# MCG-NJU/MotionRAG

Hardware: AMD Instinct MI355X
Metric: denoise_step_frames_per_sec (higher is better)
Workload: dtype bf16

## Files before the change

### motionrag_amd/csrc/gemm_w4.hip

```cpp
#include "gemm_common.h"

namespace {

__device__ __forceinline__ int lane_id_here() {
  int l;
  asm volatile("v_mbcnt_lo_u32_b32 %0, -1, 0\n\tv_mbcnt_hi_u32_b32 %0, -1, %0" : "=v"(l));
  return l;
}
__device__ __forceinline__ int opaque_sign(int x) {
  asm volatile("" : "+v"(x));
  return x;
}

template <int EPI>
__device__ __forceinline__ void epilogue_w4(const GemmP& p, char* smem, f32x4 (&acc)[8][8], const long long bm0, const long long bn0, const int wave, const int wrow0,
                                            const int wcol0, const long long Mend) {
  constexpr bool HAS_R = (EPI == MRAG_EPI_GATE_RESID || EPI == MRAG_EPI_RESID), HAS_G = (EPI == MRAG_EPI_GATE_RESID), QK = (EPI == MRAG_EPI_QKNORM_ROPE);
  const int lane = lane_id_here();
  const int frag_row = opaque_sign(lane & 15), frag_q = lane >> 4;
  const long long n0 = bn0 + wcol0 + frag_q * 4;
  const long long m0 = bm0 + wrow0;
  long long g_b = 0, g_pos = 0;
  if constexpr (HAS_G || QK) {
    g_b = m0 / p.rows_per_batch;
    g_pos = m0 - g_b * p.rows_per_batch;
  }
  if (m0 >= Mend || bn0 + wcol0 >= p.N) return;
  const int mrows = (int)(Mend - m0 < 128 ? Mend - m0 : 128);
  bool fast = p.staged && bn0 + wcol0 + 128 <= p.N;
  if constexpr (HAS_G) fast = fast && g_pos + mrows - 1 < p.rows_per_batch && ((g_pos < p.split) == (g_pos + mrows - 1 < p.split));
  auto add_resid = [&](u32x2 out, const u32x2 r2) __attribute__((always_inline)) -> u32x2 {
    out[0] = pack_bf2(__uint_as_float(out[0] << 16) + __uint_as_float(r2[0] << 16), __uint_as_float(out[0] & 0xffff0000u) + __uint_as_float(r2[0] & 0xffff0000u));
    out[1] = pack_bf2(__uint_as_float(out[1] << 16) + __uint_as_float(r2[1] << 16), __uint_as_float(out[1] & 0xffff0000u) + __uint_as_float(r2[1] & 0xffff0000u));
    return out;
  };
  auto acc_math = [&](const int i, const int j, const u32x2 b2, const u32x2 g2) __attribute__((always_inline)) -> u32x2 {
    float v[4] = {acc[i][j][0], acc[i][j][1], acc[i][j][2], acc[i][j][3]};
    v[0] += __uint_as_float(b2[0] << 16); v[1] += __uint_as_float(b2[0] & 0xffff0000u);
    v[2] += __uint_as_float(b2[1] << 16); v[3] += __uint_as_float(b2[1] & 0xffff0000u);
    if constexpr (EPI == MRAG_EPI_GELU_TANH) {
      const f32x2 lo = gelu_tanh_f2(f32x2{v[0], v[1]}), hi = gelu_tanh_f2(f32x2{v[2], v[3]});
      v[0] = lo[0]; v[1] = lo[1]; v[2] = hi[0]; v[3] = hi[1];
    } else {
#pragma unroll
      for (int e = 0; e < 4; ++e) v[e] = epi_act<EPI>(v[e]);
    }
    if constexpr (HAS_G) {
      v[0] *= __uint_as_float(g2[0] << 16); v[1] *= __uint_as_float(g2[0] & 0xffff0000u);
      v[2] *= __uint_as_float(g2[1] << 16); v[3] *= __uint_as_float(g2[1] & 0xffff0000u);
    }
    if constexpr (EPI == MRAG_EPI_RESID) {
#pragma unroll
      for (int e = 0; e < 4; ++e) v[e] *= p.acc_scale;
    }
    return u32x2{pack_bf2(v[0], v[1]), pack_bf2(v[2], v[3])};
  };
  if (fast) {
    u32x2 bias[8], gate[8];
#pragma unroll
    for (int j = 0; j < 8; ++j) {
      bias[j] = p.bias ? *(const u32x2*)(p.bias + n0 + 16 * j) : u32x2{0u, 0u};
      if constexpr (HAS_G) gate[j] = *(const u32x2*)((g_pos < p.split ? p.gate0 : p.gate1) + g_b * p.gate_stride + n0 + 16 * j);
      else gate[j] = u32x2{0u, 0u};
    }
    const int r4 = lane >> 4, chunk = opaque_sign(lane & 15);
    const bf16_t* rbase = HAS_R ? p.resid + m0 * p.ldr + n0 : nullptr;
    bf16_t* cbase = p.C + (m0 + r4) * p.ldc + (bn0 + wcol0 + chunk * 8);
    char* wput = smem + 131072 + wave * 8192 + frag_row * 256 + (frag_q & 1) * 8;
    const char* wget = smem + 131072 + wave * 8192 + r4 * 256;
    const int xput = frag_q >> 1;
    int qk_which = 2;
    bool has_rope = false;
    const bf16_t *gm = nullptr, *bt = nullptr;
    float gam[8], bet[8];
    f32x4 qk_tab[QK ? 3 : 1][4];
    unsigned qk_video = 0;
    auto qk_fetch = [&](const int st) __attribute__((always_inline)) {
      if constexpr (QK) {
        const int row = 4 * st + r4;
        long long pos = g_pos + (row < mrows ? row : mrows - 1);
        while (pos >= p.rows_per_batch) pos -= p.rows_per_batch;
        const int rp = (int)pos - p.rope_text_len;
        if (rp >= 0) qk_video |= 1u << st;
        const long long ro = (long long)opaque_sign(rp > 0 ? rp : 0) * 64 + opaque_sign(chunk & 7) * 8;
        f32x4(&dst)[4] = qk_tab[st % 3];
        dst[0] = *(const f32x4*)(p.rcos + ro); dst[1] = *(const f32x4*)(p.rcos + ro + 4);
        dst[2] = *(const f32x4*)(p.rsin + ro); dst[3] = *(const f32x4*)(p.rsin + ro + 4);
      }
    };
    if constexpr (QK) {
      qk_which = p.qk_first + (int)((bn0 + wcol0) / p.qk_D);
      has_rope = p.rcos != nullptr && qk_which < 2;
#pragma unroll
      for (int e = 0; e < 8; ++e) { gam[e] = 1.f; bet[e] = 0.f; }
      if (qk_which < 2) {
        gm = qk_which ? p.kg : p.qg;
        bt = qk_which ? p.kb : p.qb;
        const int d0 = (chunk & 7) * 8;
        if (gm) {
          const u32x4 graw = *(const u32x4*)(gm + d0);
#pragma unroll
          for (int e = 0; e < 4; ++e) { gam[2 * e] = __uint_as_float(graw[e] << 16); gam[2 * e + 1] = __uint_as_float(graw[e] & 0xffff0000u); }
          if (bt) {
            const u32x4 braw = *(const u32x4*)(bt + d0);
#pragma unroll
            for (int e = 0; e < 4; ++e) { bet[2 * e] = __uint_as_float(braw[e] << 16); bet[2 * e + 1] = __uint_as_float(braw[e] & 0xffff0000u); }
          }
        }
      }
      if (has_rope) { qk_fetch(0); qk_fetch(1); qk_fetch(2); }
    }
    constexpr int RD = 2;
    u32x2 rr[RD][8];
    auto fetch = [&](const int i, const int slot) __attribute__((always_inline)) {
      if constexpr (HAS_R) {
        const int row = 16 * i + frag_row;
        const bf16_t* rrow = rbase + (long long)(row < mrows ? row : mrows - 1) * p.ldr;
#pragma unroll
        for (int j = 0; j < 8; ++j) rr[slot][j] = *(const u32x2*)(rrow + 16 * j);
      }
    };
    auto put = [&](const int i) __attribute__((always_inline)) {
#pragma unroll
      for (int j = 0; j < 8; ++j) {
        u32x2 out = acc_math(i, j, bias[j], gate[j]);
        if constexpr (HAS_R) out = add_resid(out, rr[i % RD][j]);
        *(u32x2*)(wput + (i & 1) * 4096 + (((2 * j + xput) ^ frag_row) * 16)) = out;
      }
    };
    auto get_store = [&](const int i) __attribute__((always_inline)) {
      u32x4 val[4];
#pragma unroll
      for (int q = 0; q < 4; ++q) val[q] = *(const u32x4*)(wget + (i & 1) * 4096 + q * 1024 + ((chunk ^ (q * 4 + r4)) * 16));
#pragma unroll
      for (int q = 0; q < 4; ++q) {
        if constexpr (QK) {
          const int st = 4 * i + q;
          if (qk_which < 2) {
            val[q] = qk_row_math(val[q], gm != nullptr, bt != nullptr, gam, bet, p.qk_eps, has_rope, (qk_video >> st) & 1u, qk_tab[st % 3], qk_which == 0 && p.q_premul != 1.0f, p.q_premul);
            if (has_rope && st + 3 < 32) qk_fetch(st + 3);
          }
        }
        if (16 * i + 4 * q + r4 < mrows) *(u32x4*)(cbase + (long long)(16 * i + 4 * q) * p.ldc) = val[q];
      }
    };
#pragma unroll
    for (int i = 0; i < RD - 1; ++i) fetch(i, i);
#pragma unroll
    for (int i = 0; i < 8; ++i) {
      __builtin_amdgcn_sched_barrier(0);
      if (i + RD - 1 < 8) fetch(i + RD - 1, (i + RD - 1) % RD);
      put(i);
      if (i > 0) get_store(i - 1);
    }
    __builtin_amdgcn_sched_barrier(0);
    get_store(7);
    return;
  }
  if constexpr (QK) return;
  auto ncol = [&](const int j) __attribute__((always_inline)) { const long long n = n0 + 16 * j; return n < p.N ? n : p.N - 4; };
#pragma unroll
  for (int i = 0; i < 8; ++i) {
    __builtin_amdgcn_sched_barrier(0);
    const long long m = m0 + i * 16 + frag_row;
    const bool mok = m < Mend;
    const long long mc = mok ? m : Mend - 1;
    const bf16_t* gate = nullptr;
    if constexpr (HAS_G) {
      long long b = g_b, pos = g_pos + (mc - m0);
      while (pos >= p.rows_per_batch) { pos -= p.rows_per_batch; ++b; }
      gate = (pos < p.split ? p.gate0 : p.gate1) + b * p.gate_stride;
    }
#pragma unroll
    for (int j = 0; j < 8; ++j) {
      const long long n = ncol(j);
      const u32x2 b2 = p.bias ? *(const u32x2*)(p.bias + n) : u32x2{0u, 0u};
      u32x2 g2 = u32x2{0u, 0u};
      if constexpr (HAS_G) g2 = *(const u32x2*)(gate + n);
      u32x2 out = acc_math(i, j, b2, g2);
      if constexpr (HAS_R) out = add_resid(out, *(const u32x2*)(p.resid + mc * p.ldr + n));
      if (mok && n0 + 16 * j < p.N) *(u32x2*)(p.C + mc * p.ldc + n) = out;
    }
  }
  __builtin_amdgcn_s_waitcnt(0x0070);
}

template <int EPI>
__device__ __forceinline__ void epilogue_w4_geglu(const GemmP& p, char* smem, f32x4 (&acc)[8][8], const long long bm0, const long long bn0, const int wave, const int wrow0,
                                                  const int wcol0) {
  const int lane = lane_id_here();
  const int frag_row = lane & 15, frag_q = lane >> 4;
  const long long m0 = bm0 + wrow0;
  if (m0 >= p.M || bn0 + wcol0 >= p.N) return;
  const int mrows = (int)(p.M - m0 < 128 ? p.M - m0 : 128);
  const long long n0 = bn0 + wcol0 + frag_q * 4;
  u32x2 bv[4], bg[4];
#pragma unroll
  for (int jj = 0; jj < 4; ++jj) {
    bv[jj] = p.bias ? *(const u32x2*)(p.bias + n0 + 32 * jj) : u32x2{0u, 0u};
    bg[jj] = p.bias ? *(const u32x2*)(p.bias + n0 + 32 * jj + 16) : u32x2{0u, 0u};
  }
  const int r8 = lane >> 3, chunk = opaque_sign(lane & 7);
  bf16_t* cbase = p.C + (m0 + r8) * p.ldc + ((bn0 + wcol0) >> 1) + chunk * 8;
  char* wput = smem + 131072 + wave * 8192 + frag_row * 128 + (frag_q & 1) * 8;
  const char* wget = smem + 131072 + wave * 8192 + r8 * 128 + ((chunk ^ r8) * 16);
  const int xput = frag_q >> 1, sw = frag_row & 7;
  auto put = [&](const int i) __attribute__((always_inline)) {
#pragma unroll
    for (int jj = 0; jj < 4; ++jj) {
      float v[4] = {acc[i][2 * jj][0], acc[i][2 * jj][1], acc[i][2 * jj][2], acc[i][2 * jj][3]};
      float g[4] = {acc[i][2 * jj + 1][0], acc[i][2 * jj + 1][1], acc[i][2 * jj + 1][2], acc[i][2 * jj + 1][3]};
      v[0] += __uint_as_float(bv[jj][0] << 16); v[1] += __uint_as_float(bv[jj][0] & 0xffff0000u);
      v[2] += __uint_as_float(bv[jj][1] << 16); v[3] += __uint_as_float(bv[jj][1] & 0xffff0000u);
      g[0] += __uint_as_float(bg[jj][0] << 16); g[1] += __uint_as_float(bg[jj][0] & 0xffff0000u);
      g[2] += __uint_as_float(bg[jj][1] << 16); g[3] += __uint_as_float(bg[jj][1] & 0xffff0000u);
      geglu4<EPI == EPI_GEGLU_TANH>(v, g);
      *(u32x2*)(wput + (i & 1) * 2048 + (((2 * jj + xput) ^ sw) * 16)) = u32x2{pack_bf2(v[0], v[1]), pack_bf2(v[2], v[3])};
    }
  };
  auto get_store = [&](const int i) __attribute__((always_inline)) {
    u32x4 val[2];
#pragma unroll
    for (int q = 0; q < 2; ++q) val[q] = *(const u32x4*)(wget + (i & 1) * 2048 + q * 1024);
#pragma unroll
    for (int q = 0; q < 2; ++q)
      if (16 * i + 8 * q + r8 < mrows) *(u32x4*)(cbase + (long long)(16 * i + 8 * q) * p.ldc) = val[q];
  };
#pragma unroll
  for (int i = 0; i < 8; ++i) {
    __builtin_amdgcn_sched_barrier(0);
    put(i);
    if (i > 0) get_store(i - 1);
  }
  __builtin_amdgcn_sched_barrier(0);
  get_store(7);
}

template <int N, class F>
__device__ __forceinline__ void static_for(F&& f) {
  if constexpr (N > 0) {
    static_for<N - 1>(f);
    f(std::integral_constant<int, N - 1>{});
  }
}

__device__ __forceinline__ void tile_coords(const GemmP& p, const int L, int& tile_m, int& tile_n) {
  const int gw = p.group_m * p.tiles_n;
  const int first_m = (L / gw) * p.group_m;
  const int gsz = min(p.tiles_m - first_m, p.group_m);
  tile_m = first_m + (L % gw) % gsz;
  tile_n = (L % gw) / gsz;
}

template <int EPI, bool WB = false>
__global__ __launch_bounds__(256) void gemm_w4_kernel(const GemmP p) {
  extern __shared__ __attribute__((aligned(16))) char smem[];
  constexpr unsigned STAGE = 65536, WOFF = 32768;
  const int lane = threadIdx.x & 63;
  const int wave_s = __builtin_amdgcn_readfirstlane(threadIdx.x >> 6), wm = wave_s >> 1, wn = wave_s & 1;
  const int tiles = p.tile_limit, nk = (int)(p.K / 64), G = (int)gridDim.x;
  auto tile_origin = [&](const int tm, long long& bm0, long long& m_end, long long& w_off) __attribute__((always_inline)) {
    if constexpr (WB) {
      const int b = tm / p.wb_tiles_m;
      bm0 = (long long)b * p.rows_per_batch + (long long)(tm - b * p.wb_tiles_m) * 256;
      m_end = (long long)(b + 1) * p.rows_per_batch;
      w_off = (long long)b * p.w_bstride;
    } else {
      bm0 = (long long)tm * 256; m_end = p.M; w_off = 0;
    }
  };
  const int slot = xcd_remap((int)blockIdx.x, G);
  unsigned voff[16];
  const bf16_t *baseA = p.A, *baseW = p.W;
  int d_r = 0, d_kt = 0;
  bool d_valid = false;
  auto cursor_set = [&](const int r) __attribute__((always_inline)) {
    const int L = r * G + slot;
    d_valid = L < tiles;
    if (!d_valid) return;
    int tm, tn;
    tile_coords(p, L, tm, tn);
    long long bm0, m_end, w_off;
    tile_origin(tm, bm0, m_end, w_off);
    const long long bn0 = (long long)tn * 256;
    const int lane_c = lane_id_here();
    const int prow = lane_c >> 3, pchk = (lane_c & 7) ^ prow;
#pragma unroll
    for (int i = 0; i < 16; ++i) {
      const int q = wave_s + 4 * i;
      long long r8 = (i < 8) ? 8 * q + prow : 8 * (q - 32) + prow;
      const long long lim = (i < 8) ? m_end - bm0 : p.N - bn0;
      r8 = r8 < lim ? r8 : lim - 1;
      voff[i] = (unsigned)((r8 * ((i < 8) ? p.lda : p.ldw) + pchk * 8) * 2);
    }
    baseA = p.A + bm0 * p.lda;
    baseW = p.W + w_off + bn0 * p.ldw;
  };
  auto advance = [&]() __attribute__((always_inline)) {
    if (!d_valid) return;
    if (d_kt + 1 < nk) { ++d_kt; return; }
    cursor_set(d_r + 1);
    if (d_valid) { ++d_r; d_kt = 0; }
  };
  const unsigned smem_u = (unsigned)(size_t)smem;
  const unsigned fr = lane & 15, fq = lane >> 4, swz = lane & 7;
  const unsigned c0 = ((fq + 0) ^ swz) * 16, c1 = ((fq + 4) ^ swz) * 16;
  const unsigned rowA = smem_u + (wm * 128 + fr) * 128, rowW = smem_u + WOFF + (wn * 128 + fr) * 128;
  f32x4 acc[8][8];
  u32x4 a0[8], w0[8], a1[8], w1[8];
#define MRAG_W4_MF(I, J, W, A) asm volatile("v_mfma_f32_16x16x32_bf16 %0, %1, %2, %0" : "+a"(acc[I][J]) : "v"(W[J]), "v"(A[I]))
#define MRAG_W4_RD(D, ADDR, OFF) asm volatile("ds_read_b128 %0, %1 offset:%2" : "=v"(D) : "v"(ADDR), "n"(OFF) : "memory")
#define MRAG_W4_LGKM0(W, A)                                                                                          \
      asm volatile("s_waitcnt lgkmcnt(0)"                                                                             \
                   : "+v"(W[0]), "+v"(W[1]), "+v"(W[2]), "+v"(W[3]), "+v"(W[4]), "+v"(W[5]), "+v"(W[6]), "+v"(W[7]),   \
                     "+v"(A[0]), "+v"(A[1]), "+v"(A[2]), "+v"(A[3]), "+v"(A[4]), "+v"(A[5]), "+v"(A[6]), "+v"(A[7])    \
                   :: "memory")
  unsigned aw1, aa1, aw0, aa0, stage_u;
  auto dma = [&](auto I) __attribute__((always_inline)) {
    constexpr int i = decltype(I)::value;
    (void)&voff;
    const bf16_t* sb = (i < 8 ? baseA : baseW) + (long long)d_kt * 64;
    const unsigned lds = stage_u + (unsigned)(wave_s + 4 * i) * 1024u;
    asm volatile("s_mov_b32 m0, %2\n\ts_nop 0\n\tglobal_load_lds_dwordx4 %0, %1" :: "v"(voff[i]), "s"(sb), "s"(lds) : "memory", "m0");
  };
  auto kstep = [&](const unsigned g, const bool counted) __attribute__((always_inline)) {
    const unsigned so = (g & 1) ? STAGE : 0u, sn = STAGE - so;
    aw1 = rowW + so + c1; aa1 = rowA + so + c1;
    aw0 = rowW + sn + c0; aa0 = rowA + sn + c0;
    stage_u = smem_u + so;
    MRAG_W4_LGKM0(w0, a0);
    static_for<32>([&](auto S) __attribute__((always_inline)) {
      constexpr int sl = decltype(S)::value, i = (2 * sl) / 8, j = (2 * sl) % 8;
      (void)&acc; (void)&w0; (void)&a0; (void)&w1; (void)&a1; (void)&aw1; (void)&aa1;
      MRAG_W4_MF(i, j, w0, a0);
      if constexpr (sl < 8) MRAG_W4_RD(w1[sl], aw1, sl * 2048);
      else if constexpr (sl < 16) MRAG_W4_RD(a1[sl - 8], aa1, (sl - 8) * 2048);
      else if constexpr (sl == 22) { MRAG_W4_LGKM0(w1, a1); asm volatile("s_barrier" ::: "memory"); }
      else if constexpr (sl >= 23 && (sl & 1)) dma(std::integral_constant<int, (sl - 23) / 2>{});
      MRAG_W4_MF(i, j + 1, w0, a0);
    });
    if (counted) asm volatile("s_waitcnt vmcnt(5)" ::: "memory");
    asm volatile("s_barrier" ::: "memory");
    static_for<32>([&](auto S) __attribute__((always_inline)) {
      constexpr int sl = decltype(S)::value, i = (2 * sl) / 8, j = (2 * sl) % 8;
      (void)&acc; (void)&w0; (void)&a0; (void)&w1; (void)&a1; (void)&aw0; (void)&aa0;
      MRAG_W4_MF(i, j, w1, a1);
      if constexpr (sl < 8) MRAG_W4_RD(w0[sl], aw0, sl * 2048);
      else if constexpr (sl < 16) MRAG_W4_RD(a0[sl - 8], aa0, (sl - 8) * 2048);
      else if constexpr (sl >= 16 && sl < 27) dma(std::integral_constant<int, sl - 11>{});
      MRAG_W4_MF(i, j + 1, w1, a1);
    });
  };
  cursor_set(0);
  if (!d_valid) return;
  stage_u = smem_u;
  static_for<16>([&](auto I) __attribute__((always_inline)) { dma(I); });
  advance();
  stage_u = smem_u + STAGE;
  static_for<16>([&](auto I) __attribute__((always_inline)) { dma(I); });
  advance();
  asm volatile("s_waitcnt vmcnt(16)\n\ts_barrier" ::: "memory");
  unsigned g = 0;
  for (int r = 0;; ++r) {
    const int L = r * G + slot;
    if (L >= tiles) break;
    aw0 = rowW + ((g & 1) ? STAGE : 0u) + c0; aa0 = rowA + ((g & 1) ? STAGE : 0u) + c0;
    static_for<8>([&](auto J) __attribute__((always_inline)) { constexpr int j = decltype(J)::value; (void)&w0; (void)&aw0; MRAG_W4_RD(w0[j], aw0, j * 2048); });
    static_for<8>([&](auto J) __attribute__((always_inline)) { constexpr int j = decltype(J)::value; (void)&a0; (void)&aa0; MRAG_W4_RD(a0[j], aa0, j * 2048); });
#pragma unroll
    for (int i = 0; i < 8; ++i)
#pragma unroll
      for (int j = 0; j < 8; ++j) acc[i][j] = f32x4{0.f, 0.f, 0.f, 0.f};
    asm volatile("s_nop 4" ::: "memory");
    for (int t = 0; t < nk; ++t, ++g) {
      kstep(g, !(t == 0 && r > 0));
      advance();
    }
    asm volatile("s_waitcnt vmcnt(0) lgkmcnt(0)\n\ts_nop 15\n\ts_nop 15\n\ts_nop 7" ::: "memory");
    int tm, tn;
    tile_coords(p, L, tm, tn);
    long long e_bm0, e_mend, e_woff;
    tile_origin(tm, e_bm0, e_mend, e_woff);
    if constexpr (is_geglu<EPI>) epilogue_w4_geglu<EPI>(p, smem, acc, e_bm0, (long long)tn * 256, wave_s, wm * 128, wn * 128);
    else epilogue_w4<EPI>(p, smem, acc, e_bm0, (long long)tn * 256, wave_s, wm * 128, wn * 128, e_mend);
  }
#undef MRAG_W4_MF
#undef MRAG_W4_RD
#undef MRAG_W4_LGKM0
}

struct TailRect { bool use = false; int limit = 0; long long r0 = 0, c0 = 0; };
inline TailRect plan_tail_rect(const GemmP& p, int epi) {
  TailRect t;
  const long long tiles = (long long)p.tiles_m * p.tiles_n;
  if (p.wb_tiles_m || !tail_rect_wanted(tiles, epi, p.tuning)) return t;
  const int rem = (int)(tiles % SK_CUS);
  const int first_m = ((p.tiles_m - 1) / p.group_m) * p.group_m, gsz = p.tiles_m - first_m;
  const int ncols = (rem + gsz - 1) / gsz;
  if (ncols > p.tiles_n) return t;
  t.use = true;
  t.limit = (int)(tiles - (long long)gsz * ncols);
  t.r0 = (long long)first_m * 256; t.c0 = (long long)(p.tiles_n - ncols) * 256;
  return t;
}

}

extern "C" int launch_w4(hipStream_t s, const GemmP& p0, int epi) {
  if (256LL * (p0.lda > p0.ldw ? p0.lda : p0.ldw) * 2 >= (1LL << 32)) return MRAG_ENOTSUP;
  GemmP p = p0;
  const bool wb = p.w_bstride != 0;
  if (wb) {
    if (epi != MRAG_EPI_NONE || p.rows_per_batch <= 0 || p.M % p.rows_per_batch != 0) return MRAG_ENOTSUP;
    p.wb_tiles_m = (int)((p.rows_per_batch + 255) / 256);
    p.tiles_m = (int)(p.M / p.rows_per_batch) * p.wb_tiles_m;
  } else {
    p.wb_tiles_m = 0;
    p.tiles_m = (int)((p.M + 255) / 256);
  }
  p.tiles_n = (int)((p.N + 255) / 256);
  p.group_m = group_m_of(p.tuning);
  const long long tiles = (long long)p.tiles_m * p.tiles_n;
  p.staged = rows_16B_aligned(p.C, p.ldc, p.resid, p.ldr);
  if (p.tuning & MRAG_GEMM_TUNE_NO_STAGED) p.staged = 0;
  const TailRect tail = plan_tail_rect(p, epi);
  p.tile_limit = tail.use ? tail.limit : (int)tiles;
  const dim3 grid((unsigned)(p.tile_limit < SK_CUS ? p.tile_limit : SK_CUS)), block(256);
  const size_t lds = 131072 + 32768;
  int rc;
  switch (epi) {
    case MRAG_EPI_NONE:
      rc = wb ? launch_dyn_lds(gemm_w4_kernel<MRAG_EPI_NONE, true>, grid, block, lds, s, p) : launch_dyn_lds(gemm_w4_kernel<MRAG_EPI_NONE>, grid, block, lds, s, p);
      break;
    case MRAG_EPI_GELU_TANH: rc = launch_dyn_lds(gemm_w4_kernel<MRAG_EPI_GELU_TANH>, grid, block, lds, s, p); break;
    case MRAG_EPI_RESID: rc = launch_dyn_lds(gemm_w4_kernel<MRAG_EPI_RESID>, grid, block, lds, s, p); break;
    case MRAG_EPI_GATE_RESID: rc = launch_dyn_lds(gemm_w4_kernel<MRAG_EPI_GATE_RESID>, grid, block, lds, s, p); break;
    case MRAG_EPI_GEGLU:
    case EPI_GEGLU_TANH:
      if (!p.staged || p.N % 128 != 0) return MRAG_ENOTSUP;
      rc = epi == MRAG_EPI_GEGLU ? launch_dyn_lds(gemm_w4_kernel<MRAG_EPI_GEGLU>, grid, block, lds, s, p) : launch_dyn_lds(gemm_w4_kernel<EPI_GEGLU_TANH>, grid, block, lds, s, p);
      break;
    case MRAG_EPI_QKNORM_ROPE:
      if (!p.staged || p.N % 128 != 0 || p.qk_D % 128 != 0) return MRAG_ENOTSUP;
      rc = launch_dyn_lds(gemm_w4_kernel<MRAG_EPI_QKNORM_ROPE>, grid, block, lds, s, p);
      break;
    default: return MRAG_ENOTSUP;
  }
  if (rc != MRAG_OK) return rc;
  MRAG_COUNT(epi == MRAG_EPI_QKNORM_ROPE ? MRAG_K_GEMM_W4_QKNORM_ROPE : (epi == MRAG_EPI_GEGLU || epi == EPI_GEGLU_TANH) ? MRAG_K_GEMM_W4_GEGLU : wb ? MRAG_K_GEMM_W4_BATCHED_W : MRAG_K_GEMM_W4);
  if (tail.use) {
    GemmP t = p0;
    t.A = p0.A + tail.r0 * p0.lda; t.W = p0.W + tail.c0 * p0.ldw; t.C = p0.C + tail.r0 * p0.ldc + tail.c0;
    if (p0.bias) t.bias = p0.bias + tail.c0;
    if (p0.resid) t.resid = p0.resid + tail.r0 * p0.ldr + tail.c0;
    t.M = p0.M - tail.r0; t.N = p0.N - tail.c0;
    rc = launch_tiled(s, t, epi, TILE_128x128, nullptr);
    if (rc != MRAG_OK) return rc;
    MRAG_COUNT(MRAG_K_GEMM_W4_TAIL_RECT);
  }
  return MRAG_OK;
}
```

Baseline: 89.15.

## Restructure W4 epilogue: row-coalesced residual loads, DPP-shared rope tables, mode-specialized paths

The fast epilogue now loads the residual in the same row-contiguous 16-byte layout used for the output stores and adds it after the LDS transpose, replacing the strided 8-byte per-fragment loads. For the QK-norm/rope epilogue, each lane loads only the cos or sin half of the table and the other half is exchanged across lanes with DPP row broadcasts, with a deeper prefetch ring. The loop is also compile-time specialized into no-norm, norm-only and norm+rope variants so the per-row branches go away. This cuts global load traffic and instruction count but adds code size, register pressure from the larger ring, and a dependency on DPP lane patterns being correct.

```diff
diff --git a/motionrag_amd/csrc/gemm_w4.hip b/motionrag_amd/csrc/gemm_w4.hip
--- a/motionrag_amd/csrc/gemm_w4.hip
+++ b/motionrag_amd/csrc/gemm_w4.hip
@@ -34,6 +34,10 @@
     out[1] = pack_bf2(__uint_as_float(out[1] << 16) + __uint_as_float(r2[1] << 16), __uint_as_float(out[1] & 0xffff0000u) + __uint_as_float(r2[1] & 0xffff0000u));
     return out;
   };
+  auto add_resid4 = [&](const u32x4 out, const u32x4 r4v) __attribute__((always_inline)) -> u32x4 {
+    const u32x2 lo = add_resid(u32x2{out[0], out[1]}, u32x2{r4v[0], r4v[1]}), hi = add_resid(u32x2{out[2], out[3]}, u32x2{r4v[2], r4v[3]});
+    return u32x4{lo[0], lo[1], hi[0], hi[1]};
+  };
   auto acc_math = [&](const int i, const int j, const u32x2 b2, const u32x2 g2) __attribute__((always_inline)) -> u32x2 {
     float v[4] = {acc[i][j][0], acc[i][j][1], acc[i][j][2], acc[i][j][3]};
     v[0] += __uint_as_float(b2[0] << 16); v[1] += __uint_as_float(b2[0] & 0xffff0000u);
@@ -64,16 +68,19 @@
       else gate[j] = u32x2{0u, 0u};
     }
     const int r4 = lane >> 4, chunk = opaque_sign(lane & 15);
-    const bf16_t* rbase = HAS_R ? p.resid + m0 * p.ldr + n0 : nullptr;
+    const bf16_t* rbase = HAS_R ? p.resid + (m0 + r4) * p.ldr + (bn0 + wcol0 + chunk * 8) : nullptr;
+    const bf16_t* rlast = HAS_R ? p.resid + (m0 + mrows - 1) * p.ldr + (bn0 + wcol0 + chunk * 8) : nullptr;
     bf16_t* cbase = p.C + (m0 + r4) * p.ldc + (bn0 + wcol0 + chunk * 8);
     char* wput = smem + 131072 + wave * 8192 + frag_row * 256 + (frag_q & 1) * 8;
     const char* wget = smem + 131072 + wave * 8192 + r4 * 256;
     const int xput = frag_q >> 1;
+    constexpr int QK_RING = 6;
     int qk_which = 2;
     bool has_rope = false;
     const bf16_t *gm = nullptr, *bt = nullptr;
     float gam[8], bet[8];
-    f32x4 qk_tab[QK ? 3 : 1][4];
+    f32x4 qk_tab[QK ? QK_RING : 1][2];
+    const float* qk_half = nullptr;
     unsigned qk_video = 0;
     auto qk_fetch = [&](const int st) __attribute__((always_inline)) {
       if constexpr (QK) {
@@ -83,9 +90,20 @@
         const int rp = (int)pos - p.rope_text_len;
         if (rp >= 0) qk_video |= 1u << st;
         const long long ro = (long long)opaque_sign(rp > 0 ? rp : 0) * 64 + opaque_sign(chunk & 7) * 8;
-        f32x4(&dst)[4] = qk_tab[st % 3];
-        dst[0] = *(const f32x4*)(p.rcos + ro); dst[1] = *(const f32x4*)(p.rcos + ro + 4);
-        dst[2] = *(const f32x4*)(p.rsin + ro); dst[3] = *(const f32x4*)(p.rsin + ro + 4);
+        f32x4(&dst)[2] = qk_tab[st % QK_RING];
+        dst[0] = *(const f32x4*)(qk_half + ro); dst[1] = *(const f32x4*)(qk_half + ro + 4);
+      }
+    };
+    auto qk_table = [&](const int st, f32x4 (&t4)[4]) __attribute__((always_inline)) {
+      if constexpr (QK) {
+#pragma unroll
+        for (int h = 0; h < 2; ++h)
+#pragma unroll
+          for (int e = 0; e < 4; ++e) {
+            const int own = __float_as_int(qk_tab[st % QK_RING][h][e]);
+            t4[h][e] = __int_as_float(__builtin_amdgcn_update_dpp(own, own, 0x128, 0xF, 0xC, false));
+            t4[2 + h][e] = __int_as_float(__builtin_amdgcn_update_dpp(own, own, 0x128, 0xF, 0x3, false));
+          }
       }
     };
     if constexpr (QK) {
@@ -108,53 +126,68 @@
           }
         }
       }
-      if (has_rope) { qk_fetch(0); qk_fetch(1); qk_fetch(2); }
-    }
-    constexpr int RD = 2;
-    u32x2 rr[RD][8];
-    auto fetch = [&](const int i, const int slot) __attribute__((always_inline)) {
+      if (has_rope) qk_half = (chunk & 8) ? p.rsin : p.rcos;
+    }
+    constexpr int RD = 3;
+    u32x4 rr[HAS_R ? RD : 1][4];
+    auto fetch = [&](const int i) __attribute__((always_inline)) {
       if constexpr (HAS_R) {
-        const int row = 16 * i + frag_row;
-        const bf16_t* rrow = rbase + (long long)(row < mrows ? row : mrows - 1) * p.ldr;
-#pragma unroll
-        for (int j = 0; j < 8; ++j) rr[slot][j] = *(const u32x2*)(rrow + 16 * j);
+#pragma unroll
+        for (int q = 0; q < 4; ++q) {
+          const int row0 = 16 * i + 4 * q;
+          const bf16_t* src = row0 + r4 < mrows ? rbase + (long long)row0 * p.ldr : rlast;
+          rr[i % RD][q] = *(const u32x4*)src;
+        }
       }
     };
     auto put = [&](const int i) __attribute__((always_inline)) {
 #pragma unroll
-      for (int j = 0; j < 8; ++j) {
-        u32x2 out = acc_math(i, j, bias[j], gate[j]);
-        if constexpr (HAS_R) out = add_resid(out, rr[i % RD][j]);
-        *(u32x2*)(wput + (i & 1) * 4096 + (((2 * j + xput) ^ frag_row) * 16)) = out;
-      }
-    };
-    auto get_store = [&](const int i) __attribute__((always_inline)) {
+      for (int j = 0; j < 8; ++j) *(u32x2*)(wput + (i & 1) * 4096 + (((2 * j + xput) ^ frag_row) * 16)) = acc_math(i, j, bias[j], gate[j]);
+    };
+    auto get_store = [&](const int i, auto MODE) __attribute__((always_inline)) {
+      constexpr int mode = decltype(MODE)::value;
       u32x4 val[4];
 #pragma unroll
       for (int q = 0; q < 4; ++q) val[q] = *(const u32x4*)(wget + (i & 1) * 4096 + q * 1024 + ((chunk ^ (q * 4 + r4)) * 16));
 #pragma unroll
       for (int q = 0; q < 4; ++q) {
-        if constexpr (QK) {
+        if constexpr (QK && mode > 0) {
           const int st = 4 * i + q;
-          if (qk_which < 2) {
-            val[q] = qk_row_math(val[q], gm != nullptr, bt != nullptr, gam, bet, p.qk_eps, has_rope, (qk_video >> st) & 1u, qk_tab[st % 3], qk_which == 0 && p.q_premul != 1.0f, p.q_premul);
-            if (has_rope && st + 3 < 32) qk_fetch(st + 3);
+          f32x4 t4[4] = {};
+          if constexpr (mode == 2) qk_table(st, t4);
+          val[q] = qk_row_math(val[q], gm != nullptr, bt != nullptr, gam, bet, p.qk_eps, mode == 2, (qk_video >> st) & 1u, t4, qk_which == 0 && p.q_premul != 1.0f, p.q_premul);
+          if constexpr (mode == 2) {
+            if (st + QK_RING < 32) qk_fetch(st + QK_RING);
           }
         }
+        if constexpr (HAS_R) val[q] = add_resid4(val[q], rr[i % RD][q]);
         if (16 * i + 4 * q + r4 < mrows) *(u32x4*)(cbase + (long long)(16 * i + 4 * q) * p.ldc) = val[q];
       }
     };
-#pragma unroll
-    for (int i = 0; i < RD - 1; ++i) fetch(i, i);
-#pragma unroll
-    for (int i = 0; i < 8; ++i) {
+    auto run = [&](auto MODE) __attribute__((always_inline)) {
+      constexpr int mode = decltype(MODE)::value;
+      if constexpr (mode == 2) {
+#pragma unroll
+        for (int st = 0; st < QK_RING; ++st) qk_fetch(st);
+      }
+      fetch(0);
+#pragma unroll
+      for (int i = 0; i < 8; ++i) {
+        __builtin_amdgcn_sched_barrier(0);
+        if (i + 1 < 8) fetch(i + 1);
+        put(i);
+        if (i > 0) get_store(i - 1, MODE);
+      }
       __builtin_amdgcn_sched_barrier(0);
-      if (i + RD - 1 < 8) fetch(i + RD - 1, (i + RD - 1) % RD);
-      put(i);
-      if (i > 0) get_store(i - 1);
-    }
-    __builtin_amdgcn_sched_barrier(0);
-    get_store(7);
+      get_store(7, MODE);
+    };
+    if constexpr (QK) {
+      if (qk_which >= 2) run(std::integral_constant<int, 0>{});
+      else if (!has_rope) run(std::integral_constant<int, 1>{});
+      else run(std::integral_constant<int, 2>{});
+    } else {
+      run(std::integral_constant<int, 0>{});
+    }
     return;
   }
   if constexpr (QK) return;
```

Result: no change. 89.90, median of 6 (+0.8%).
